# antonilo/unsupervised_detection

Measured on NVIDIA H100. Metric: frame-pairs/sec adversarial train step 256x448, higher is better.
Workload: dtype bf16

## Files before the change

include/cis_b200.h:

```cpp
#ifndef CIS_B200_H_
#define CIS_B200_H_
#include <stdint.h>
#include <stddef.h>

#ifdef __cplusplus
extern "C" {
#endif

typedef void* cis_stream_t;

enum { CIS_OK = 0, CIS_ERR_BAD_ARG = 1, CIS_ERR_UNSUPPORTED = 2, CIS_ERR_CUDA = 3 };
enum { CIS_ACT_NONE = 0, CIS_ACT_ELU = 1, CIS_ACT_LEAKY = 2 };
enum { CIS_MAX_TAPS = 49, CIS_MAX_SRC = 4 };

typedef struct {
  const void* ptr;
  int32_t pitch;
  int32_t c_off;
  int32_t chunks;
  int32_t n_mod;
} CisSrc;

typedef struct {
  int32_t N, H, W;
  int32_t OH, OW;
  int32_t sh, sw;
  int32_t ntaps;
  int16_t dh[CIS_MAX_TAPS];
  int16_t dw[CIS_MAX_TAPS];
  int32_t nsrc;
  CisSrc src[CIS_MAX_SRC];
  const void* wpack;
  int32_t K_pad;
  int32_t BN;
  int32_t n_tiles;
  const float* bias;
  int32_t act;
  float alpha;
  int32_t DH, DW;
  int32_t osh, osw, oa, ob;
  void* out;
  int32_t out_pitch, out_coff, out_ch;
  float* outf;
  int32_t outf_pitch, outf_coff, outf_ch;
  const void* add_pre;
  int32_t add_pre_pitch, add_pre_coff;
  const float* addf_pre;
  int32_t addf_pitch, addf_coff;
  const void* add_post;
  int32_t add_post_pitch, add_post_coff;
  int32_t mode;
  int32_t halo;
  int32_t dil;
  int32_t MT;
  int32_t hoy, hox;
  int32_t ey, ex;
  int32_t splits;
  float* sk_scratch;
  int32_t* sk_counters;
  int32_t nph;
  int32_t ph_tap[5];
  int32_t sk_cluster;
  int32_t nsub;
  struct {
    int32_t tap0, ntaps;
    int32_t hoy, hox;
    int32_t OH, OW, oa, ob;
    const void* wpack;
  } sub[4];
  int32_t nwg;
  int32_t thin;
} CisConv;

typedef struct {
  int32_t N, H, W, OH, OW, sh, sw, ntaps;
  int16_t dh[CIS_MAX_TAPS];
  int16_t dw[CIS_MAX_TAPS];
  int32_t nsrc;
  CisSrc src[CIS_MAX_SRC];
  const void* g;
  int32_t g_pitch, g_coff, g_chunks;
  float* dwp;
  int32_t Cout;
  int32_t K_pad;
  int32_t splits;
  int32_t tma;
  int32_t nh;
  int32_t nwg;
} CisWgrad;

const char* cis_last_error(void);
int cis_version(void);
uint32_t cis_crc32c(uint32_t crc, const void* data, size_t n);
int cis_host_resize_bilinear_legacy(const float* src, int32_t H, int32_t W, int32_t C, float* dst, int32_t OH, int32_t OW);
int cis_host_bgr8_to_rgb_resized(const unsigned char* bgr, int32_t H, int32_t W, float* dst, int32_t OH, int32_t OW);

int cis_conv_igemm(const CisConv* d, cis_stream_t stream);
int cis_conv_s2_phase_plan(const CisConv* d, CisConv* h, int16_t* wk);
int cis_set_persist_mode(int mode);
int cis_conv_wgrad(const CisWgrad* d, cis_stream_t stream);

int cis_pack_weights(const float* w, const int32_t* kmap, int32_t K_pad, int32_t rows, int32_t cout, int32_t sn, const int32_t* nmap,
                     void* wp, cis_stream_t stream);
int cis_pack_weights_tiled(const float* w, const int32_t* kmap, int32_t cin8, int32_t ntaps, int32_t n_tiles, int32_t BN, int32_t cout,
                           int32_t sn, const int32_t* nmap, void* out, int32_t thin, cis_stream_t stream);
int cis_unpack_wgrad(const float* dwp, const int32_t* kmap, int32_t K_pad, int32_t cout, int32_t nsplit, float* dw, const float* colpart,
                     int32_t nblocks, int32_t nch, float* db, int32_t layout, cis_stream_t stream);
int cis_bn_fold(const float* w, const float* bias, const float* gamma, const float* beta, int64_t nw, int32_t cout, float* w_eff,
                float* b_eff, cis_stream_t stream);
int cis_bn_chain(const float* w, const float* bias, const float* gamma, float* dw_eff_to_dw, const float* db_eff, int64_t nw,
                 int32_t cout, float* dbias, float* dgamma, float* dbeta, cis_stream_t stream);

enum { CIS_JOB_PACK = 0, CIS_JOB_PACK_TILED = 1, CIS_JOB_UNPACK = 2, CIS_JOB_BN_FOLD = 3, CIS_JOB_BN_CHAIN = 4 };
typedef struct {
  int32_t kind;
  int32_t i[8];
  int64_t n;
  const void* p[8];
} CisParamJob;
int cis_param_multi(const CisParamJob* jobs_dev, int32_t njobs, int32_t total_blocks, cis_stream_t stream);

int cis_dact_mul(void* g, int32_t g_pitch, int32_t g_coff, const void* y, int32_t y_pitch, int32_t y_coff, const void* res,
                 int32_t res_pitch, int32_t res_coff, int64_t npix, int32_t chunks, int32_t act, float alpha, cis_stream_t stream);
int cis_add_slice(void* dst, int32_t dst_pitch, int32_t dst_coff, const void* src, int32_t src_pitch, int32_t src_coff,
                  int64_t npix_dst, int32_t chunks, int32_t reps, int32_t accumulate, cis_stream_t stream);
int cis_colsum(const void* g, int32_t g_pitch, int32_t g_coff, int64_t npix, int32_t nch, float* part, int32_t nblocks, cis_stream_t stream);

int cis_zero(void* ptr, int64_t nbytes, cis_stream_t stream);

int cis_dact_colsum(void* g, int32_t g_pitch, int32_t g_coff, const void* y, int32_t y_pitch, int32_t y_coff, const void* res,
                    int32_t res_pitch, int32_t res_coff, int64_t npix, int32_t nch, int32_t act, float alpha, float* part, int32_t nblocks,
                    cis_stream_t stream);

int cis_resize_bilinear_bf16(const void* src, int32_t s_pitch, int32_t s_coff, int32_t N, int32_t H, int32_t W, void* dst,
                             int32_t d_pitch, int32_t d_coff, int32_t OH, int32_t OW, int32_t chunks, cis_stream_t stream);
int cis_resize_concat_bf16(const CisSrc* srcs, int32_t nsrc, int32_t N, int32_t H, int32_t W, void* dst, int32_t d_pitch, int32_t d_coff,
                           int32_t OH, int32_t OW, cis_stream_t stream);
int cis_resize_concat_bf16_bwd(const void* ddst, int32_t d_pitch, int32_t d_coff, int32_t N, int32_t OH, int32_t OW, const CisSrc* grads,
                               const int32_t* want, const int32_t* accumulate, int32_t nsrc, int32_t H, int32_t W, cis_stream_t stream);
int cis_resize_bilinear_bf16_bwd(const void* ddst, int32_t d_pitch, int32_t d_coff, int32_t N, int32_t OH, int32_t OW, void* dsrc,
                                 int32_t s_pitch, int32_t s_coff, int32_t H, int32_t W, int32_t chunks, int32_t accumulate,
                                 cis_stream_t stream);
int cis_resize_bilinear_f32(const float* src, int32_t N, int32_t H, int32_t W, int32_t C, float* dst, int32_t OH, int32_t OW,
                            float scale, cis_stream_t stream);
int cis_upsample_nn2x(const void* src, int32_t N, int32_t H, int32_t W, int32_t pitch, void* dst, cis_stream_t stream);
int cis_upsample_nn2x_bwd(const void* ddst, int32_t N, int32_t H, int32_t W, int32_t pitch, void* dsrc, int32_t accumulate,
                          cis_stream_t stream);
int cis_crop_resize_bilinear_f32(const float* src, int32_t Hs, int32_t Ws, int32_t C, int32_t y0, int32_t x0, int32_t ch, int32_t cw, float* dst,
                                 int32_t OH, int32_t OW, cis_stream_t stream);
int cis_crop_resize_flow_f32(const float* src, int32_t Hs, int32_t Ws, int32_t y0, int32_t x0, int32_t ch, int32_t cw, float* dst, int32_t OH,
                             int32_t OW, float s0, float s1, cis_stream_t stream);
int cis_resize_nn_f32(const float* src, int32_t N, int32_t H, int32_t W, int32_t C, float* dst, int32_t OH, int32_t OW,
                      cis_stream_t stream);
enum { CIS_RESIZE_BILINEAR = 0, CIS_RESIZE_NEAREST = 1 };
int cis_resize_f32(const float* src, int32_t N, int32_t H, int32_t W, int32_t C, float* dst, int32_t OH, int32_t OW, int32_t method,
                   int32_t align_corners, cis_stream_t stream);
int cis_resize_f32_bwd(const float* ddst, int32_t N, int32_t OH, int32_t OW, int32_t C, int32_t H, int32_t W, float* dsrc, int32_t method,
                       int32_t align_corners, cis_stream_t stream);

int cis_warp_costvol(const void* c1, int32_t c1_pitch, int32_t c1_coff, const void* c2, int32_t c2_pitch, int32_t c2_coff,
                     const float* flow, float flow_scale, int32_t B, int32_t h, int32_t w, int32_t C, void* out, int32_t out_pitch,
                     int32_t out_coff, cis_stream_t stream);
int cis_warp_costvol_r(const void* c1, int32_t c1_pitch, int32_t c1_coff, const void* c2, int32_t c2_pitch, int32_t c2_coff,
                       const float* flow, float flow_scale, int32_t B, int32_t h, int32_t w, int32_t C, void* out, int32_t out_pitch,
                       int32_t out_coff, int32_t search_range, cis_stream_t stream);
int cis_dense_image_warp(const void* img, int32_t pitch, int32_t coff, const float* flow, float flow_scale, int32_t B, int32_t h,
                         int32_t w, int32_t C, void* out, int32_t out_pitch, cis_stream_t stream);

int cis_pack_f32_to_bf16(const float* src, int64_t npix, int32_t C, float offset, void* dst, int32_t d_pitch, int32_t d_coff,
                         cis_stream_t stream);
int cis_flow_stats(const float* flow, int32_t B, int64_t hw, double* stats, cis_stream_t stream);
int cis_pack_generator_input(const float* image, const float* flow, const double* stats, int32_t B, int64_t hw, void* dst,
                             cis_stream_t stream);
int cis_flow_standardize(const float* flow, const double* stats, int32_t B, int64_t hw, float* out, cis_stream_t stream);
int cis_flow_standardize_bwd(const float* y, const float* dy, const double* stats, int32_t B, int64_t hw, double* scratch, float* dx,
                             cis_stream_t stream);
int cis_masked_epe(const float* pred, const float* gt, const float* mask, int32_t B, int64_t hw, double* scratch, double* out,
                   cis_stream_t stream);

int cis_mask_apply(const float* flow, const float* mask, int32_t B, int64_t hw, void* dst, cis_stream_t stream);
int cis_box_masks(float* mask, int32_t B, int32_t H, int32_t W, int32_t lo_h, int32_t hi_h, int32_t lo_w, int32_t hi_w, int64_t sample_offset,
                  const long long* step, uint64_t seed, cis_stream_t stream);
int cis_charbonnier_sum(const float* gt, const float* pred, const float* mask, int32_t B, int64_t hw, int32_t C, int32_t mask_c, float cbn,
// ... 93 lines not shown
```

unsupervised_detection_b200/_lib.py:

```python
import ctypes as C
import os

_HERE = os.path.dirname(os.path.abspath(__file__))
LIB_PATH = os.path.join(_HERE, os.environ.get('CIS_LIB_NAME', 'libcis_b200.so'))

MAX_TAPS, MAX_SRC = 49, 4
ACT_NONE, ACT_ELU, ACT_LEAKY = 0, 1, 2
RESIZE_BILINEAR, RESIZE_NEAREST = 0, 1


class CisSrc(C.Structure):
    _fields_ = [('ptr', C.c_void_p), ('pitch', C.c_int32), ('c_off', C.c_int32), ('chunks', C.c_int32), ('n_mod', C.c_int32)]


class CisParamJob(C.Structure):
    _fields_ = [('kind', C.c_int32), ('i', C.c_int32 * 8), ('n', C.c_int64), ('p', C.c_void_p * 8)]


JOB_PACK, JOB_PACK_TILED, JOB_UNPACK, JOB_BN_FOLD, JOB_BN_CHAIN = range(5)


class CisSub(C.Structure):
    _fields_ = [('tap0', C.c_int32), ('ntaps', C.c_int32), ('hoy', C.c_int32), ('hox', C.c_int32), ('OH', C.c_int32), ('OW', C.c_int32),
                ('oa', C.c_int32), ('ob', C.c_int32), ('wpack', C.c_void_p)]
# ... 34 lines not shown
    _fields_ = [('flow', C.c_void_p * 5), ('grad', C.c_void_p * 5), ('pitch', C.c_int32 * 5), ('c_off', C.c_int32 * 5),
                ('accumulate', C.c_int32 * 5), ('weight', C.c_float * 5)]


class CisFlowAug(C.Structure):
    _fields_ = [('scale', C.c_float * 2), ('rotate', C.c_float * 2), ('translate', C.c_float * 2), ('rel_scale', C.c_float * 2),
                ('rel_rotate', C.c_float * 2), ('rel_translate', C.c_float * 2), ('color', C.c_float * 2), ('contrast', C.c_float * 2),
                ('brightness', C.c_float), ('gamma', C.c_float * 2), ('noise', C.c_float * 2)]


FLOW_AUG_ROW = 32


_i32, _i64, _f32, _p, _u64 = C.c_int32, C.c_int64, C.c_float, C.c_void_p, C.c_uint64

_PROTOS = {
    'cis_conv_igemm': [C.POINTER(CisConv)],
    'cis_conv_wgrad': [C.POINTER(CisWgrad)],
    'cis_pack_weights': [_p, _p, _i32, _i32, _i32, _i32, _p, _p],
    'cis_pack_weights_tiled': [_p, _p, _i32, _i32, _i32, _i32, _i32, _i32, _p, _p, _i32],
    'cis_unpack_wgrad': [_p, _p, _i32, _i32, _i32, _p, _p, _i32, _i32, _p, _i32],
    'cis_bn_fold': [_p, _p, _p, _p, _i64, _i32, _p, _p],
    'cis_param_multi': [_p, _i32, _i32],
    'cis_bn_chain': [_p, _p, _p, _p, _p, _i64, _i32, _p, _p, _p],
    'cis_dact_mul': [_p, _i32, _i32, _p, _i32, _i32, _p, _i32, _i32, _i64, _i32, _i32, _f32],
    'cis_add_slice': [_p, _i32, _i32, _p, _i32, _i32, _i64, _i32, _i32, _i32],
    'cis_colsum': [_p, _i32, _i32, _i64, _i32, _p, _i32],
    'cis_zero': [_p, _i64],
    'cis_dact_colsum': [_p, _i32, _i32, _p, _i32, _i32, _p, _i32, _i32, _i64, _i32, _i32, _f32, _p, _i32],
    'cis_resize_bilinear_bf16': [_p, _i32, _i32, _i32, _i32, _i32, _p, _i32, _i32, _i32, _i32, _i32],
    'cis_resize_concat_bf16': [C.POINTER(CisSrc), _i32, _i32, _i32, _i32, _p, _i32, _i32, _i32, _i32],
    'cis_resize_concat_bf16_bwd': [_p, _i32, _i32, _i32, _i32, _i32, C.POINTER(CisSrc), C.POINTER(C.c_int32), C.POINTER(C.c_int32), _i32, _i32, _i32],
    'cis_resize_bilinear_bf16_bwd': [_p, _i32, _i32, _i32, _i32, _i32, _p, _i32, _i32, _i32, _i32, _i32, _i32],
    'cis_resize_bilinear_f32': [_p, _i32, _i32, _i32, _i32, _p, _i32, _i32, _f32],
    'cis_upsample_nn2x': [_p, _i32, _i32, _i32, _i32, _p],
    'cis_upsample_nn2x_bwd': [_p, _i32, _i32, _i32, _i32, _p, _i32],
    'cis_crop_resize_bilinear_f32': [_p, _i32, _i32, _i32, _i32, _i32, _i32, _i32, _p, _i32, _i32],
    'cis_crop_resize_flow_f32': [_p, _i32, _i32, _i32, _i32, _i32, _i32, _p, _i32, _i32, _f32, _f32],
    'cis_resize_nn_f32': [_p, _i32, _i32, _i32, _i32, _p, _i32, _i32],
    'cis_resize_f32': [_p, _i32, _i32, _i32, _i32, _p, _i32, _i32, _i32, _i32],
    'cis_resize_f32_bwd': [_p, _i32, _i32, _i32, _i32, _i32, _i32, _p, _i32, _i32],
    'cis_flow_standardize': [_p, _p, _i32, _i64, _p],
    'cis_flow_standardize_bwd': [_p, _p, _p, _i32, _i64, _p, _p],
    'cis_masked_epe': [_p, _p, _p, _i32, _i64, _p, _p],
    'cis_warp_costvol': [_p, _i32, _i32, _p, _i32, _i32, _p, _f32, _i32, _i32, _i32, _i32, _p, _i32, _i32],
    'cis_dense_image_warp': [_p, _i32, _i32, _p, _f32, _i32, _i32, _i32, _i32, _p, _i32],
    'cis_pack_f32_to_bf16': [_p, _i64, _i32, _f32, _p, _i32, _i32],
    'cis_flow_stats': [_p, _i32, _i64, _p],
    'cis_pack_generator_input': [_p, _p, _p, _i32, _i64, _p],
    'cis_mask_apply': [_p, _p, _i32, _i64, _p],
    'cis_box_masks': [_p, _i32, _i32, _i32, _i32, _i32, _i32, _i32, _i64, _p, _u64],
    'cis_charbonnier_sum': [_p, _p, _p, _i32, _i64, _i32, _i32, _f32, _p],
    'cis_cis_loss_fwd': [_p, _p, _p, _i32, _i32, _i32, _i32, _i32, _f32, _p, _p],
    'cis_cis_loss_reduce': [_p, _i32, _i32, _i64, _f32, _p, _p],
    'cis_cis_loss_bwd': [_p, _p, _p, _p, _p, _i32, _i32, _i32, _i32, _i32, _f32, _i32, _p, _p],
    'cis_resize_f32_bwd_to_bf16': [_p, _i32, _i32, _i32, _i32, _i32, _i32, _p, _i32],
    'cis_mask_bwd': [_p, _p, _p, _p, _i32, _i64, _p],
    'cis_abs_sum': [_p, _i64, _p],
    'cis_grad_avg_abs': [_p, _p, _i32, _p],
    'cis_clip_adam': [_p, _p, _p, _p, _i64, _f32, _f32, _f32, _f32, _f32, _f32, _p, _p, _i32, _u64],
    'cis_cast_f32_to_bf16': [_p, _i64, _p],
    'cis_cast_bf16_to_f32': [_p, _i64, _i32, _i32, _i32, _p],
    'cis_cast_bf16_to_f32_scaled': [_p, _i64, _i32, _i32, _i32, _f32, _p],
    'cis_charbonnier_bwd': [_p, _p, _p, _i32, _i64, _i32, _i32, _f32, _p, _p, _p, _p],
    'cis_dense_image_warp_bwd': [_p, _i32, _i32, _p, _f32, _i32, _i32, _i32, _i32, _p, _p, _p, _p],
    'cis_cost_volume_bwd': [_p, _i32, _i32, _p, _i32, _i32, _p, _i32, _i32, _i32, _i32, _p, _p, _p],
    'cis_resize_f32_bwd_to_bf16_scaled': [_p, _i32, _i32, _i32, _i32, _i32, _i32, _p, _i32, _f32],
    'cis_warp_costvol_bwd': [_p, _i32, _i32, _p, _i32, _i32, _p, _f32, _i32, _i32, _i32, _i32, _p, _i32, _i32, _p, _i32, _i32, _p, _i32, _i32,
                             _p, _i32, _i32, _i32, _p, _p, _p],
    'cis_parity_split_bf16': [_p, _i32, _i32, _i32, _i32, _i32, _i32, _p, _i32],
    'cis_flow_multiscale_loss': [C.POINTER(CisFlowPyr), _p, _i32, _i32, _i32, _i32, _i32, _f32, _f32, _i32, _f32, _f32, _p, _p],
    'cis_flow_multiscale_loss_bwd': [C.POINTER(CisFlowPyr), _p, _i32, _i32, _i32, _i32, _i32, _f32, _f32, _i32, _f32, _f32],
    'cis_adam_l2': [_p, _p, _p, _p, _i64, _p, _i32, _f32, _p, _f32, _f32, _f32, _p],
    'cis_unsup_flow_loss': [_p, _p, _p, _i32, _i32, _i32, _p, _p, _p, _p, _p],
    'cis_unsup_flow_loss_bwd': [_p, _p, _p, _i32, _i32, _i32, _p, _p, _f32, _f32, _p],
    'cis_flow_aug_params': [C.POINTER(CisFlowAug), _i32, _i32, _i32, _i64, _p, _u64, _p],
    'cis_flow_augment': [_p, _p, _p, _p, _i32, _i32, _i32, _p, _p, _p],
    'cis_warp_costvol_r': [_p, _i32, _i32, _p, _i32, _i32, _p, _f32, _i32, _i32, _i32, _i32, _p, _i32, _i32, _i32],
    'cis_cost_volume_bwd_r': [_p, _i32, _i32, _p, _i32, _i32, _p, _i32, _i32, _i32, _i32, _p, _p, _p, _i32],
    'cis_warp_costvol_bwd_r': [_p, _i32, _i32, _p, _i32, _i32, _p, _f32, _i32, _i32, _i32, _i32, _p, _i32, _i32, _p, _i32, _i32, _p, _i32, _i32,
                               _p, _i32, _i32, _i32, _p, _p, _p, _i32],
}
EXPORTS = sorted(list(_PROTOS) + ['cis_last_error', 'cis_version', 'cis_set_persist_mode', 'cis_crc32c', 'cis_host_resize_bilinear_legacy',
                                  'cis_host_bgr8_to_rgb_resized', 'cis_conv_s2_phase_plan'])

_lib = None


def load():
    global _lib
    if _lib is None:
        if not os.path.exists(LIB_PATH):
            raise RuntimeError('libcis_b200.so not built: run `python -c "import __graft_entry__ as g; g.build()"` '
                               '(no CPU fallback exists for the product path)')
        lib = C.CDLL(LIB_PATH)
        lib.cis_last_error.restype = C.c_char_p
        lib.cis_version.restype = C.c_int
        lib.cis_set_persist_mode.argtypes = [C.c_int]
        lib.cis_set_persist_mode.restype = C.c_int
        lib.cis_crc32c.argtypes = [C.c_uint32, C.c_void_p, C.c_size_t]
        lib.cis_crc32c.restype = C.c_uint32
        lib.cis_host_resize_bilinear_legacy.argtypes = [C.c_void_p, C.c_int32, C.c_int32, C.c_int32, C.c_void_p, C.c_int32, C.c_int32]
        lib.cis_host_resize_bilinear_legacy.restype = C.c_int
        lib.cis_host_bgr8_to_rgb_resized.argtypes = [C.c_void_p, C.c_int32, C.c_int32, C.c_void_p, C.c_int32, C.c_int32]
        lib.cis_host_bgr8_to_rgb_resized.restype = C.c_int
        lib.cis_conv_s2_phase_plan.argtypes = [C.POINTER(CisConv), C.POINTER(CisConv), C.POINTER(C.c_int16)]
        lib.cis_conv_s2_phase_plan.restype = C.c_int
        for name, args in _PROTOS.items():
            fn = getattr(lib, name)
            fn.argtypes = list(args) + [C.c_void_p]
            fn.restype = C.c_int
        _lib = lib
    return _lib


def check(rc, what=''):
    if rc != 0:
        raise RuntimeError('libcis_b200 %s failed (code %d): %s' % (what, rc, load().cis_last_error().decode()))


def call(name, *args):
    check(getattr(load(), name)(*args), name)
```

unsupervised_detection_b200/csrc/conv_igemm.cu:

```cuda
#include "ptx.cuh"
#include "../../include/cis_b200.h"
#include "common.cuh"
#include <cuda.h>
#include <stdlib.h>
#include <string.h>


namespace cis {

#ifdef CIS_TRACE
__device__ unsigned long long* g_trace = nullptr;
__device__ int g_trace_cap = 0;
#define CIS_TRACE_AT(slot)                                                                                         \
  do {                                                                                                             \
    if (g_trace && blockIdx.x == 0 && blockIdx.y == 0 && blockIdx.z == 0 && (slot) < g_trace_cap) g_trace[(slot)] = clock64(); \
  } while (0)
#else
#define CIS_TRACE_AT(slot) ((void)0)
#endif

static constexpr int kBM = 128;
static constexpr int kBK = 64;
static constexpr int kAStage = kBM * 128;
static constexpr int kThreads = 256;
// ... 1284 lines not shown
      const uint32_t st = tile_base + s * kWStage;
#pragma unroll
      for (int r = rl; r < 64; r += nprod >> 3) {
        const int g = (kb0 + it) * 64 + r;
        const bool rv = g < M;
        int n = 0, h0 = 0, w0 = 0;
        if (rv) {
          const int ow = g % p.OW;
          const int t = g / p.OW;
          h0 = (t % p.OH) * p.sh;
          n = t / p.OH;
          w0 = ow * p.sw;
        }
        const uint32_t dst = st + r * 128 + sw_off;
#pragma unroll
        for (int u = 0; u < 2; ++u) {
          const bool ok = rv && avalid[u];
          const size_t off = ok ? ((size_t)g * p.g_pitch + p.g_coff + (u * 8 + j) * 8) : 0;
          cp_async16(dst + u * kWTile, gp + off, ok ? 16u : 0u);
        }
#pragma unroll
        for (int u = 0; u < 2; ++u) {
          const int h = h0 + bdh[u], w = w0 + bdw[u];
          const bool ok = rv && bvalid[u] && (unsigned)h < (unsigned)p.H && (unsigned)w < (unsigned)p.W;
          const int ne = bnmod[u] ? (n % bnmod[u]) : n;
          const size_t off = ok ? ((size_t)((ne * p.H + h) * p.W + w) * bpitch[u] + bcoff[u]) : 0;
          cp_async16(dst + (2 + u) * kWTile, bptr[u] + off, ok ? 16u : 0u);
        }
      }
      cp_async_commit();
      if (it >= S - 1) {
        cp_async_wait<S - 1>();
        fence_proxy_async();
        mbar_arrive(bar_full + 8 * ((it - (S - 1)) % S));
      }
    }
    cp_async_wait<0>();
    fence_proxy_async();
    for (int it = nkb > S - 1 ? nkb - (S - 1) : 0; it < nkb; ++it) mbar_arrive(bar_full + 8 * (it % S));

    }
    mbar_wait(bar_accum, 0);
    const int co = (warp & 3) * 32 + lane;
    const uint32_t t_row = tile_base + (uint32_t)co * 16;
    const int c_lo = mma_warp == 8 ? (warp >> 2) * 64 : 0, c_hi = mma_warp == 8 ? c_lo + 64 : 128;
    const int kcol0 = blockIdx.x * 128;
#pragma unroll 1
    for (int c0 = c_lo; c0 < c_hi; c0 += 16) {
      float v[16];
      acc_ld16(t_row + (uint32_t)c0 * kAccColBytes, v);
      if (co < p.Cout && kcol0 + c0 < p.K_pad) {
        float4* o = reinterpret_cast<float4*>(p.dwp) + (size_t)blockIdx.y * p.Cout * (p.K_pad / 4) + (size_t)((kcol0 + c0) / 4) * p.Cout + co;
        o[0] = make_float4(v[0], v[1], v[2], v[3]);
        o[p.Cout] = make_float4(v[4], v[5], v[6], v[7]);
        o[2 * p.Cout] = make_float4(v[8], v[9], v[10], v[11]);
        o[3 * p.Cout] = make_float4(v[12], v[13], v[14], v[15]);
      }
    }
  } else {
    const int wtid = tid - mma_warp * 32;
    float acc[128];
    for (int it = 0; it < nkb; ++it) {
      const int s = it % S;
      mbar_wait(bar_full + 8 * s, (uint32_t)((it / S) & 1));
      const uint32_t st = tile_base + s * kWStage;
      const uint32_t alo = desc_lo(st, kWTile), blo = desc_lo(st + 2 * kWTile, kWTile), dhi = desc_hi(1024);
      wg_fence();
#pragma unroll
      for (int k = 0; k < 4; ++k) mma128<128, 1, 1>(acc, alo + 128 * k, dhi, blo + 128 * k, dhi, (uint32_t)kWTile >> 4, (uint32_t)((it | k) != 0));
      wg_commit();
      wg_wait<0>();
      if (wtid == 0) mbar_arrive(bar_empty + 8 * s);
    }
    acc_store<128>(acc, tile_base, wtid);
    mbar_arrive(bar_accum);
  }
}


static constexpr int kWHMaxStages = 6;
struct WgradHaloMaps {
  CUtensorMap g;
  CUtensorMap x[CIS_MAX_SRC];
};
template <int NH> struct WgradHaloCfg {
  static_assert(NH == 16 || NH == 32 || NH == 64, "NH is 16, 32 or 64 output channels");
  static constexpr int kPairs = kMaxAccCols / NH;
  static constexpr uint32_t kGRow = 2 * NH;
  static constexpr uint32_t kGTile = 64 * kGRow;
  static constexpr uint32_t kLayout = NH == 64 ? 1u : NH == 32 ? 2u : 3u;
};

template <int NH, int NWG>
__device__ __forceinline__ void wgrad_halo_wg_pairs(int w, int npairs, int cout, int& qa, int& np, int& hf) {
  constexpr int P = WgradHaloCfg<NH>::kPairs;
  const int nhalf = cout > 64 ? 2 : 1;
  if (NWG == 2 && nhalf == 2) {
    qa = blockIdx.z * P;
    np = min(P, npairs - qa);
    hf = w;
    return;
  }
  const int q0 = (blockIdx.z / nhalf) * (NWG * P);
  const int cnt = min(NWG * P, npairs - q0);
  const int h = NWG == 2 ? (cnt + 1) / 2 : cnt;
  qa = q0 + (w ? h : 0);
  np = w ? cnt - h : h;
  hf = blockIdx.z % nhalf;
}

template <int NH, int NWG>
__global__ void __launch_bounds__(128 * (1 + NWG)) conv_wgrad_halo_kernel(const __grid_constant__ CisWgrad p, const __grid_constant__ WgradHaloMaps maps,
                                                                          const int Wh, const int Hh, const int hoy, const int hox,
                                                                          const int stage_bytes, const int S) {
  using Cfg = WgradHaloCfg<NH>;
  constexpr int P = Cfg::kPairs;
  extern __shared__ uint8_t smem_raw[];
  __shared__ uint64_t bars[2 * kWHMaxStages + 1];
  __shared__ int s_off[CIS_MAX_TAPS + 1];
  const uint32_t tile_base = (smem_u32(smem_raw) + 1023u) & ~1023u;
  const uint32_t bar_full = smem_u32(&bars[0]);
  const uint32_t bar_empty = smem_u32(&bars[kWHMaxStages]);
  const uint32_t bar_accum = smem_u32(&bars[2 * kWHMaxStages]);
  const int tid = threadIdx.x, warp = tid >> 5, lane = tid & 31;
  pdl_launch_dependents();
  if (tid < p.ntaps) s_off[tid] = (p.dh[tid] - hoy) * Wh + (p.dw[tid] - hox);
  if (tid == p.ntaps) s_off[tid] = 0;
  const bool wg_halves = NWG == 2 && p.Cout > 64;
  const int ng = wg_halves ? 2 : 1;
  const int halo_bytes = stage_bytes - ng * (int)Cfg::kGTile;
  const int tiles_x = (p.OW + 7) / 8, tiles_y = (p.OH + 7) / 8;
  const int nkb_total = p.N * tiles_x * tiles_y;
  const int per = (nkb_total + (int)gridDim.y - 1) / (int)gridDim.y;
  const int kb0 = blockIdx.y * per;
  const int nkb = min(per, nkb_total - kb0);
  if (nkb <= 0) return;
  int m_chunks = 0;
  for (int i = 0; i < p.nsrc; ++i) m_chunks += p.src[i].chunks;
  const int nch64 = (m_chunks + 7) / 8;
  const int npairs = (p.ntaps + 1) / 2;
  const int c64 = blockIdx.x;

  if (tid == 128) {
    for (int s = 0; s < S; ++s) {
      mbar_init(bar_full + 8 * s, 1);
      mbar_init(bar_empty + 8 * s, NWG);
    }
    mbar_init(bar_accum, 128 * NWG);
    fence_mbar_init();
  }
  pdl_wait();
  __syncthreads();

  if (warp < 4) {
    if (tid == 0) {
      int c = c64 * 8, si = 0;
      while (si < p.nsrc - 1 && c >= p.src[si].chunks) {
        c -= p.src[si].chunks;
        ++si;
      }
      int nm = p.src[0].n_mod;
      if (si == 1) nm = p.src[1].n_mod;
      if (si == 2) nm = p.src[2].n_mod;
      if (si == 3) nm = p.src[3].n_mod;
      int qa, np, hf0;
      wgrad_halo_wg_pairs<NH, NWG>(0, npairs, p.Cout, qa, np, hf0);
      const int tpi = tiles_x * tiles_y;
      for (int it = 0; it < nkb; ++it) {
        const int s = it % S;
        mbar_wait(bar_empty + 8 * s, (uint32_t)(((it / S) & 1) ^ 1));
        const int kb = kb0 + it;
        const int n = kb / tpi, r = kb - n * tpi;
        const int ty = r / tiles_x, tx = r - ty * tiles_x;
        const uint32_t st = tile_base + s * stage_bytes, bar = bar_full + 8 * s;
        mbar_expect_tx(bar, (uint32_t)(Wh * Hh * 128 + ng * (int)Cfg::kGTile));
        tma_load_4d(st, &maps.x[si], bar, c * 8, tx * 8 + hox, ty * 8 + hoy, nm ? (n % nm) : n);
        for (int h = 0; h < ng; ++h)
          tma_load_4d(st + halo_bytes + h * Cfg::kGTile, &maps.g, bar, (hf0 + h) * 64, tx * 8, ty * 8, n);
      }
    }
    __syncwarp();
    mbar_wait(bar_accum, 0);
    const int r = warp * 32 + lane;
    const int cch = r & 63;
    const uint32_t t_row = tile_base + (uint32_t)r * 16;
    for (int w = 0; w < NWG; ++w) {
      int qa, np, hf;
      wgrad_halo_wg_pairs<NH, NWG>(w, npairs, p.Cout, qa, np, hf);
      for (int q = 0; q < np; ++q) {
        const int t = 2 * (qa + q) + (r >> 6);
        if (t >= p.ntaps) continue;
        const size_t kcol = ((size_t)t * nch64 + c64) * 64 + cch;
#pragma unroll 1
        for (int c0 = 0; c0 < NH && hf * 64 + c0 < p.Cout; c0 += 16) {
          float v[16];
          acc_ld16(t_row + (uint32_t)((w * P + q) * NH + c0) * kAccColBytes, v);
          for (int e = 0; e < 16; ++e) {
            const int co = hf * 64 + c0 + e;
            if (co < p.Cout) p.dwp[((size_t)blockIdx.y * p.Cout + co) * p.K_pad + kcol] = v[e];
          }
        }
      }
    }
  } else {
    const int wg = NWG > 1 ? (warp - 4) >> 2 : 0;
    const int wtid = tid - 128 * (1 + wg);
    int qa, np, hf;
    wgrad_halo_wg_pairs<NH, NWG>(wg, npairs, p.Cout, qa, np, hf);
    np = __shfl_sync(0xffffffffu, np, 0);
    float acc[P][NH];
    const uint32_t ahi = desc_hi((uint32_t)(Wh * 128));
    const uint32_t bhi = (((8 * Cfg::kGRow) >> 4) & 0x3FFF) | (Cfg::kLayout << 30);
    const uint32_t kstep = (uint32_t)(2 * Wh * 128) >> 4;
    const uint32_t g_off = (uint32_t)halo_bytes + (wg_halves ? (uint32_t)wg * Cfg::kGTile : 0u);
    for (int it = 0; it < nkb; ++it) {
      const int s = it % S;
      mbar_wait(bar_full + 8 * s, (uint32_t)((it / S) & 1));
      const uint32_t st = tile_base + s * stage_bytes;
      const uint32_t blo0 = desc_lo(st + g_off, Cfg::kGTile);
      wg_fence();
#pragma unroll
      for (int q = 0; q < P; ++q) {
        if (q < np) {
          const int o0 = s_off[2 * (qa + q)], o1 = s_off[2 * (qa + q) + 1];
          const uint32_t lbo = (uint32_t)((o1 > o0 ? o1 - o0 : 1) * 128);
          const uint32_t alo0 = desc_lo(st + (uint32_t)(o0 * 128), lbo);
#pragma unroll
          for (int k = 0; k < 4; ++k)
            mma128<NH, 1, 1>(acc[q], alo0 + k * kstep, ahi, blo0 + Cfg::kGRow * k, bhi, lbo >> 4, (uint32_t)((it | k) != 0));
        }
      }
      wg_commit();
      wg_wait<0>();
      if (wtid == 0) mbar_arrive(bar_empty + 8 * s);
    }
    if constexpr (NWG > 1) asm volatile("bar.sync 1, %0;" ::"n"(128 * NWG) : "memory");
#pragma unroll
    for (int q = 0; q < P; ++q)
      if (q < np) acc_store<NH>(acc[q], tile_base + (uint32_t)((wg * P + q) * NH) * kAccColBytes, wtid);
    mbar_arrive(bar_accum);
  }
}

}

using namespace cis;

static bool pdl_enabled() {
  static const bool on = !(getenv("CIS_PDL") && atoi(getenv("CIS_PDL")) == 0);
  return on;
}
template <typename... KArgs, typename... Args>
static cudaError_t launch_pdl(void (*kern)(KArgs...), dim3 grid, dim3 block, size_t smem, cudaStream_t st, Args... args) {
  cudaLaunchConfig_t cfg;
  memset(&cfg, 0, sizeof(cfg));
  cfg.gridDim = grid;
  cfg.blockDim = block;
  cfg.dynamicSmemBytes = smem;
  cfg.stream = st;
  cudaLaunchAttribute attr[1];
  attr[0].id = cudaLaunchAttributeProgrammaticStreamSerialization;
  attr[0].val.programmaticStreamSerializationAllowed = 1;
  cfg.attrs = attr;
  cfg.numAttrs = pdl_enabled() ? 1 : 0;
  return cudaLaunchKernelEx(&cfg, kern, KArgs(args)...);
}

template <typename... KArgs, typename... Args>
static cudaError_t launch_pdl_zcluster(void (*kern)(KArgs...), dim3 grid, dim3 block, size_t smem, cudaStream_t st, int cz, Args... args) {
  cudaLaunchConfig_t cfg;
  memset(&cfg, 0, sizeof(cfg));
  cfg.gridDim = grid;
  cfg.blockDim = block;
  cfg.dynamicSmemBytes = smem;
  cfg.stream = st;
  cudaLaunchAttribute attr[2];
  attr[0].id = cudaLaunchAttributeClusterDimension;
  attr[0].val.clusterDim.x = 1;
  attr[0].val.clusterDim.y = 1;
  attr[0].val.clusterDim.z = cz;
  attr[1].id = cudaLaunchAttributeProgrammaticStreamSerialization;
  attr[1].val.programmaticStreamSerializationAllowed = 1;
// ... 298 lines not shown
    const long ncta = (long)g->N * tiles_x * tiles_y * g->n_tiles;
    const int cps = max(1, min(225 * 1024 / smem, 4));
    const double t_mma = MT * 2.0 * BN * nst * 0.25, t_mem = (double)kb * nst / 40.0 + halo / 40.0;
    const double t_cta = fmax(t_mma, t_mem) + (4000.0 + 1500.0 * MT) / cps;
    const double cost = (double)((ncta + (long)nsm * cps - 1) / ((long)nsm * cps)) * cps * t_cta / fmin((double)cps, fmax(1.0, (double)ncta / nsm));
    if (!best_mt || cost < best - 1e-9) {
      best = cost;
      best_mt = MT;
    }
  }
  if (!best_mt || (long)g->N * tiles_x * ((g->OH + 16 * best_mt - 1) / (16 * best_mt)) * g->n_tiles < 296) return false;
  h->halo = 1;
  h->sh = h->sw = 1;
  h->dil = 1;
  h->MT = best_mt;
  h->nwg = 1;
  h->hoy = hoy;
  h->hox = hox;
  h->ey = ey;
  h->ex = ex;
  h->nph = 4;
  for (int q = 0; q < 5; ++q) h->ph_tap[q] = bounds[q];
  h->thin = thin;
  h->splits = 0;
  h->sk_cluster = 0;
  for (int s = 0; s < nst; ++s)
    for (int j = 0; j < 2; ++j) {
      const int i = thin == 8 ? 2 * s + j : s;
      wk[2 * s + j] = (int16_t)(thin == 8 ? (i < nt ? order[i] * 8 : g->K_pad) : order[i] * 16 + 8 * j);
    }
  return true;
}
extern "C" int cis_conv_s2_phase_plan(const CisConv* d, CisConv* h, int16_t* wk) {
  return d && h && wk && !d->halo && s2_phase_plan(d, h, wk) ? 1 : 0;
}

extern "C" int cis_conv_igemm(const CisConv* d, cis_stream_t stream) {
  if (!d || d->ntaps < 1 || d->ntaps > CIS_MAX_TAPS || d->nsrc < 1 || d->nsrc > CIS_MAX_SRC || d->K_pad % 64 != 0 || d->K_pad <= 0 ||
      d->n_tiles < 1 || !d->wpack)
    return cis_set_error(CIS_ERR_BAD_ARG, "cis_conv_igemm: bad descriptor");
  int chunks = 0;
  for (int i = 0; i < d->nsrc; ++i) {
    if ((d->src[i].pitch | d->src[i].c_off) & 7) return cis_set_error(CIS_ERR_BAD_ARG, "cis_conv_igemm: source pitch/c_off must be multiples of 8");
    chunks += d->src[i].chunks;
  }
  if (d->ntaps * chunks * 8 > d->K_pad) return cis_set_error(CIS_ERR_BAD_ARG, "cis_conv_igemm: K_pad smaller than taps*channels");
  if (d->mode == 1 && !d->outf) return cis_set_error(CIS_ERR_BAD_ARG, "cis_conv_igemm: mode 1 needs outf");
  if ((d->add_pre || d->add_post) && (((d->add_pre_pitch | d->add_pre_coff | d->add_post_pitch | d->add_post_coff | d->out_ch) & 7) != 0))
    return cis_set_error(CIS_ERR_BAD_ARG, "cis_conv_igemm: residual slices must be 8-channel aligned");
  cudaStream_t st = (cudaStream_t)stream;
  if (d->halo) {
    if (d->MT < 1 || d->MT > 4 || d->MT * d->BN > kMaxAccCols || d->nwg < 0 || d->nwg > 2 || (d->nwg == 2 && d->BN < 64) || d->dil < 1 ||
        d->sh != 1 || d->sw != 1 || d->ey < 0 || d->ex < 0 ||
        (d->dil > 1 && (d->OH != d->H || d->OW != d->W)) || (d->nph > 1 && (d->nph != 4 || d->dil != 1 || d->ph_tap[0] != 0 || d->ph_tap[4] != d->ntaps)))
      return cis_set_error(CIS_ERR_BAD_ARG, "cis_conv_igemm(halo): bad tile parameters");
    switch (d->BN) {
      case 16: return launch_halo<16, 1>(d, st);
      case 32: return launch_halo<32, 1>(d, st);
      case 64: return d->nwg == 2 ? launch_halo<64, 2>(d, st) : launch_halo<64, 1>(d, st);
      case 128: return d->nwg == 2 ? launch_halo<128, 2>(d, st) : launch_halo<128, 1>(d, st);
      default: return cis_set_error(CIS_ERR_UNSUPPORTED, "cis_conv_igemm: BN must be 16/32/64/128");
    }
  }
  CisConv h;
  int16_t wk[2 * CIS_MAX_TAPS];
  if (s2_phase_plan(d, &h, wk)) {
    switch (h.BN) {
      case 16: return launch_halo<16, 1>(&h, st, wk);
      case 32: return launch_halo<32, 1>(&h, st, wk);
      case 64: return launch_halo<64, 1>(&h, st, wk);
      case 128: return launch_halo<128, 1>(&h, st, wk);
    }
  }
  switch (d->BN) {
    case 16: return launch_fwd<16>(d, st);
    case 32: return launch_fwd<32>(d, st);
    case 64: return launch_fwd<64>(d, st);
    case 128: return launch_fwd<128>(d, st);
    default: return cis_set_error(CIS_ERR_UNSUPPORTED, "cis_conv_igemm: BN must be 16/32/64/128");
  }
}

template <int NH, int NWG>
static int launch_wgrad_halo_t(const CisWgrad* d, cudaStream_t st, int nch64, int Wh, int Hh, int hoy, int hox, int halo_bytes) {
  using Cfg = WgradHaloCfg<NH>;
  const bool wg_halves = NWG == 2 && d->Cout > 64;
  const int stage = halo_bytes + (wg_halves ? 2 : 1) * (int)Cfg::kGTile;
  const int npairs = (d->ntaps + 1) / 2, nhalf = d->Cout > 64 ? 2 : 1;
  const int gz = wg_halves ? (npairs + Cfg::kPairs - 1) / Cfg::kPairs : nhalf * ((npairs + NWG * Cfg::kPairs - 1) / (NWG * Cfg::kPairs));
  int S = (200 * 1024) / stage;
  if (S > kWHMaxStages) S = kWHMaxStages;
  if (S < 2) return cis_set_error(CIS_ERR_UNSUPPORTED, "cis_conv_wgrad(halo): halo does not fit shared memory");
  int smem = S * stage + 1024;
  const int acc_smem = NWG * kMaxAccCols * (int)kAccColBytes + 1024;
  if (smem < acc_smem) smem = acc_smem;
  static int attr_smem = 0;
  if (smem > attr_smem) {
    cudaError_t e = cudaFuncSetAttribute(conv_wgrad_halo_kernel<NH, NWG>, cudaFuncAttributeMaxDynamicSharedMemorySize, smem);
    if (e != cudaSuccess) return cis_set_cuda_error(e, "cudaFuncSetAttribute(conv_wgrad_halo)");
    attr_smem = smem;
  }
  WgradHaloMaps maps;
  memset(&maps, 0, sizeof(maps));
  CisSrc gs;
  gs.ptr = d->g; gs.pitch = d->g_pitch; gs.c_off = d->g_coff; gs.chunks = d->g_chunks; gs.n_mod = 0;
  const CUtensorMapSwizzle gswz = NH == 64 ? CU_TENSOR_MAP_SWIZZLE_128B : NH == 32 ? CU_TENSOR_MAP_SWIZZLE_64B : CU_TENSOR_MAP_SWIZZLE_32B;
  bool ok = encode_src_map(&maps.g, gs, d->N, d->OH, d->OW, 8, 8, 1, 0, 0, 1, NH, gswz);
  for (int i = 0; ok && i < d->nsrc; ++i) ok = encode_src_map(&maps.x[i], d->src[i], d->N, d->H, d->W, Wh, Hh);
  if (!ok) return cis_set_error(CIS_ERR_CUDA, "cis_conv_wgrad(halo): cuTensorMapEncodeTiled failed / unavailable");
  dim3 grid(nch64, d->splits, gz);
  cudaError_t le = launch_pdl(conv_wgrad_halo_kernel<NH, NWG>, grid, dim3(128 * (1 + NWG)), (size_t)smem, st, *d, maps, Wh, Hh, hoy, hox, stage, S);
  if (le != cudaSuccess) return cis_set_cuda_error(le, "launch(conv_wgrad_halo)");
  return cis_check_launch("conv_wgrad_halo");
}

static int launch_wgrad_halo(const CisWgrad* d, cudaStream_t st) {
  if (d->sh != 1 || d->sw != 1) return cis_set_error(CIS_ERR_BAD_ARG, "cis_conv_wgrad(halo): needs a stride-1 layer");
  int chunks = 0;
  for (int i = 0; i < d->nsrc; ++i) chunks += d->src[i].chunks;
  for (int i = 0; i < d->nsrc - 1; ++i)
    if (d->src[i].chunks % 8) return cis_set_error(CIS_ERR_BAD_ARG, "cis_conv_wgrad(halo): needs 64-channel aligned concat sources");
  const int nch64 = (chunks + 7) / 8;
  int hoy = d->dh[0], hox = d->dw[0], my = d->dh[0], mx = d->dw[0];
  for (int t = 1; t < d->ntaps; ++t) {
    if (d->dh[t] < hoy) hoy = d->dh[t];
    if (d->dw[t] < hox) hox = d->dw[t];
    if (d->dh[t] > my) my = d->dh[t];
    if (d->dw[t] > mx) mx = d->dw[t];
  }
  for (int t = 1; t < d->ntaps; ++t)
    if ((d->dh[t] - hoy) * 1024 + (d->dw[t] - hox) <= (d->dh[t - 1] - hoy) * 1024 + (d->dw[t - 1] - hox))
      return cis_set_error(CIS_ERR_BAD_ARG, "cis_conv_wgrad(halo): taps must be listed in increasing row-major order");
  const int Wh = 8 + (mx - hox), Hh = 8 + (my - hoy);
  if (Wh > 256 || Hh > 256) return cis_set_error(CIS_ERR_UNSUPPORTED, "cis_conv_wgrad(halo): tap extent too large");
  if (d->K_pad < d->ntaps * nch64 * 64) return cis_set_error(CIS_ERR_BAD_ARG, "cis_conv_wgrad(halo): K_pad smaller than taps * 64-channel groups");
  const int nh = d->nh ? d->nh : 64, nwg = d->nwg ? d->nwg : 1;
  if ((nh != 16 && nh != 32 && nh != 64) || nh < (d->Cout > 64 ? 64 : (d->Cout + 15) / 16 * 16) || nwg < 1 || nwg > 2)
    return cis_set_error(CIS_ERR_BAD_ARG, "cis_conv_wgrad(halo): nh must be 16/32/64 and cover Cout (64 above 64), nwg 1 or 2");
  const int halo_bytes = (Wh * Hh * 128 + 1023) & ~1023;
  switch (nh * 4 + nwg) {
    case 16 * 4 + 1: return launch_wgrad_halo_t<16, 1>(d, st, nch64, Wh, Hh, hoy, hox, halo_bytes);
    case 16 * 4 + 2: return launch_wgrad_halo_t<16, 2>(d, st, nch64, Wh, Hh, hoy, hox, halo_bytes);
    case 32 * 4 + 1: return launch_wgrad_halo_t<32, 1>(d, st, nch64, Wh, Hh, hoy, hox, halo_bytes);
    case 32 * 4 + 2: return launch_wgrad_halo_t<32, 2>(d, st, nch64, Wh, Hh, hoy, hox, halo_bytes);
    case 64 * 4 + 1: return launch_wgrad_halo_t<64, 1>(d, st, nch64, Wh, Hh, hoy, hox, halo_bytes);
    default: return launch_wgrad_halo_t<64, 2>(d, st, nch64, Wh, Hh, hoy, hox, halo_bytes);
  }
}

extern "C" int cis_conv_wgrad(const CisWgrad* d, cis_stream_t stream) {
  if (!d || d->ntaps < 1 || d->ntaps > CIS_MAX_TAPS || d->nsrc < 1 || d->nsrc > CIS_MAX_SRC || d->K_pad % 64 != 0 || d->Cout < 1 ||
      d->Cout > 128 || d->splits < 1 || !d->g || !d->dwp)
    return cis_set_error(CIS_ERR_BAD_ARG, "cis_conv_wgrad: bad descriptor");
  {
    const long M = (long)d->N * d->OH * d->OW;
    const long nkb_total = d->tma ? (long)d->N * ((d->OW + 7) / 8) * ((d->OH + 7) / 8) : (M + 63) / 64;
    const long per = (nkb_total + d->splits - 1) / d->splits;
    if ((long)(d->splits - 1) * per >= nkb_total) return cis_set_error(CIS_ERR_BAD_ARG, "cis_conv_wgrad: a split would own no reduction block");
  }
  if (d->tma == 2) return launch_wgrad_halo(d, (cudaStream_t)stream);
  static bool attr_set = false;
  if (!attr_set) {
    cudaError_t e = cudaFuncSetAttribute(conv_wgrad_kernel, cudaFuncAttributeMaxDynamicSharedMemorySize, kWSmem);
    if (e != cudaSuccess) return cis_set_cuda_error(e, "cudaFuncSetAttribute(conv_wgrad)");
    attr_set = true;
  }
  WgradMaps maps;
  memset(&maps, 0, sizeof(maps));
  if (d->tma) {
    if (d->sh != 1 || d->sw != 1) return cis_set_error(CIS_ERR_BAD_ARG, "cis_conv_wgrad: TMA path needs a stride-1 layer");
    for (int i = 0; i < d->nsrc - 1; ++i)
      if (d->src[i].chunks % 8) return cis_set_error(CIS_ERR_BAD_ARG, "cis_conv_wgrad: TMA path needs 64-channel aligned concat sources");
    CisSrc gs;
    gs.ptr = d->g; gs.pitch = d->g_pitch; gs.c_off = d->g_coff; gs.chunks = d->g_chunks; gs.n_mod = 0;
    bool ok = encode_src_map(&maps.g, gs, d->N, d->OH, d->OW, 8, 8);
    for (int i = 0; ok && i < d->nsrc; ++i) ok = encode_src_map(&maps.x[i], d->src[i], d->N, d->H, d->W, 8, 8);
    if (!ok) return cis_set_error(CIS_ERR_CUDA, "cis_conv_wgrad: cuTensorMapEncodeTiled failed / unavailable");
  }
  dim3 grid((d->K_pad + 127) / 128, d->splits);
  cudaError_t le = launch_pdl(conv_wgrad_kernel, grid, dim3(d->tma ? kThreads : kGThreads), kWSmem, (cudaStream_t)stream, *d, maps);
  if (le != cudaSuccess) return cis_set_cuda_error(le, "launch(conv_wgrad)");
  return cis_check_launch("conv_wgrad");
}
```

Measured before the change: 661.7.

## Route stride-2 weight-gradient convs through phase-split TMA halo kernel

Adds a stride-2 phase decomposition for weight-gradient convolutions. Taps are regrouped by input parity into four phase planes, each loaded by its own strided TMA tensor map into the halo kernel, which writes results through a per-tap column remap. Stride-2 layers that previously fell to the generic non-TMA wgrad kernel now run on the stride-1 halo path when the plan's constraints are met. This costs four times the halo shared memory per stage, plus padding taps when a phase has an odd tap count.

```diff
diff --git a/include/cis_b200.h b/include/cis_b200.h
--- a/include/cis_b200.h
+++ b/include/cis_b200.h
@@ -99,6 +99,7 @@
 int cis_conv_s2_phase_plan(const CisConv* d, CisConv* h, int16_t* wk);
 int cis_set_persist_mode(int mode);
 int cis_conv_wgrad(const CisWgrad* d, cis_stream_t stream);
+int cis_conv_wgrad_s2_phase_plan(const CisWgrad* d, CisWgrad* h, int16_t* kcol, int32_t* ph_tap);
 
 int cis_pack_weights(const float* w, const int32_t* kmap, int32_t K_pad, int32_t rows, int32_t cout, int32_t sn, const int32_t* nmap,
                      void* wp, cis_stream_t stream);
diff --git a/unsupervised_detection_b200/_lib.py b/unsupervised_detection_b200/_lib.py
--- a/unsupervised_detection_b200/_lib.py
+++ b/unsupervised_detection_b200/_lib.py
@@ -140,7 +140,8 @@
                                _p, _i32, _i32, _i32, _p, _p, _p, _i32],
 }
 EXPORTS = sorted(list(_PROTOS) + ['cis_last_error', 'cis_version', 'cis_set_persist_mode', 'cis_crc32c', 'cis_host_resize_bilinear_legacy',
-                                  'cis_host_bgr8_to_rgb_resized', 'cis_conv_s2_phase_plan'])
+                                  'cis_host_bgr8_to_rgb_resized', 'cis_conv_s2_phase_plan',
+                                  'cis_conv_wgrad_s2_phase_plan'])
 
 _lib = None
 
@@ -164,6 +165,8 @@
         lib.cis_host_bgr8_to_rgb_resized.restype = C.c_int
         lib.cis_conv_s2_phase_plan.argtypes = [C.POINTER(CisConv), C.POINTER(CisConv), C.POINTER(C.c_int16)]
         lib.cis_conv_s2_phase_plan.restype = C.c_int
+        lib.cis_conv_wgrad_s2_phase_plan.argtypes = [C.POINTER(CisWgrad), C.POINTER(CisWgrad), C.POINTER(C.c_int16), C.POINTER(C.c_int32)]
+        lib.cis_conv_wgrad_s2_phase_plan.restype = C.c_int
         for name, args in _PROTOS.items():
             fn = getattr(lib, name)
             fn.argtypes = list(args) + [C.c_void_p]
diff --git a/unsupervised_detection_b200/csrc/conv_igemm.cu b/unsupervised_detection_b200/csrc/conv_igemm.cu
--- a/unsupervised_detection_b200/csrc/conv_igemm.cu
+++ b/unsupervised_detection_b200/csrc/conv_igemm.cu
@@ -1390,6 +1390,9 @@
 struct WgradHaloMaps {
   CUtensorMap g;
   CUtensorMap x[CIS_MAX_SRC];
+  int16_t kcol[CIS_MAX_TAPS];
+  int32_t nph;
+  int32_t ph_tap[5];
 };
 template <int NH> struct WgradHaloCfg {
   static_assert(NH == 16 || NH == 32 || NH == 64, "NH is 16, 32 or 64 output channels");
@@ -1420,7 +1423,7 @@
 template <int NH, int NWG>
 __global__ void __launch_bounds__(128 * (1 + NWG)) conv_wgrad_halo_kernel(const __grid_constant__ CisWgrad p, const __grid_constant__ WgradHaloMaps maps,
                                                                           const int Wh, const int Hh, const int hoy, const int hox,
-                                                                          const int stage_bytes, const int S) {
+                                                                          const int stage_bytes, const int S, const int plane) {
   using Cfg = WgradHaloCfg<NH>;
   constexpr int P = Cfg::kPairs;
   extern __shared__ uint8_t smem_raw[];
@@ -1432,7 +1435,12 @@
   const uint32_t bar_accum = smem_u32(&bars[2 * kWHMaxStages]);
   const int tid = threadIdx.x, warp = tid >> 5, lane = tid & 31;
   pdl_launch_dependents();
-  if (tid < p.ntaps) s_off[tid] = (p.dh[tid] - hoy) * Wh + (p.dw[tid] - hox);
+  const int nph = maps.nph > 1 ? 4 : 1;
+  if (tid < p.ntaps) {
+    int ph = 0;
+    while (ph < nph - 1 && tid >= maps.ph_tap[ph + 1]) ++ph;
+    s_off[tid] = nph > 1 && maps.kcol[tid] < 0 ? 0 : ph * (plane >> 7) + (p.dh[tid] - hoy) * Wh + (p.dw[tid] - hox);
+  }
   if (tid == p.ntaps) s_off[tid] = 0;
   const bool wg_halves = NWG == 2 && p.Cout > 64;
   const int ng = wg_halves ? 2 : 1;
@@ -1481,8 +1489,9 @@
         const int n = kb / tpi, r = kb - n * tpi;
         const int ty = r / tiles_x, tx = r - ty * tiles_x;
         const uint32_t st = tile_base + s * stage_bytes, bar = bar_full + 8 * s;
-        mbar_expect_tx(bar, (uint32_t)(Wh * Hh * 128 + ng * (int)Cfg::kGTile));
-        tma_load_4d(st, &maps.x[si], bar, c * 8, tx * 8 + hox, ty * 8 + hoy, nm ? (n % nm) : n);
+        mbar_expect_tx(bar, (uint32_t)(nph * Wh * Hh * 128 + ng * (int)Cfg::kGTile));
+        for (int ph = 0; ph < nph; ++ph)
+          tma_load_4d(st + ph * plane, &maps.x[si * nph + ph], bar, c * 8, tx * 8 + hox, ty * 8 + hoy, nm ? (n % nm) : n);
         for (int h = 0; h < ng; ++h)
           tma_load_4d(st + halo_bytes + h * Cfg::kGTile, &maps.g, bar, (hf0 + h) * 64, tx * 8, ty * 8, n);
       }
@@ -1498,14 +1507,23 @@
       for (int q = 0; q < np; ++q) {
         const int t = 2 * (qa + q) + (r >> 6);
         if (t >= p.ntaps) continue;
-        const size_t kcol = ((size_t)t * nch64 + c64) * 64 + cch;
+        size_t base = (size_t)blockIdx.y * p.Cout * p.K_pad, cstride = p.K_pad;
+        if (nph > 1) {
+          const int ch = c64 * 64 + cch;
+          if (maps.kcol[t] < 0 || ch >= m_chunks * 8) continue;
+          const int k = maps.kcol[t] + ch;
+          base += (size_t)(k >> 2) * p.Cout * 4 + (k & 3);
+          cstride = 4;
+        } else {
+          base += ((size_t)t * nch64 + c64) * 64 + cch;
+        }
 #pragma unroll 1
         for (int c0 = 0; c0 < NH && hf * 64 + c0 < p.Cout; c0 += 16) {
           float v[16];
           acc_ld16(t_row + (uint32_t)((w * P + q) * NH + c0) * kAccColBytes, v);
           for (int e = 0; e < 16; ++e) {
             const int co = hf * 64 + c0 + e;
-            if (co < p.Cout) p.dwp[((size_t)blockIdx.y * p.Cout + co) * p.K_pad + kcol] = v[e];
+            if (co < p.Cout) p.dwp[base + (size_t)co * cstride] = v[e];
           }
         }
       }
@@ -1970,7 +1988,8 @@
 }
 
 template <int NH, int NWG>
-static int launch_wgrad_halo_t(const CisWgrad* d, cudaStream_t st, int nch64, int Wh, int Hh, int hoy, int hox, int halo_bytes) {
+static int launch_wgrad_halo_t(const CisWgrad* d, cudaStream_t st, int nch64, int Wh, int Hh, int hoy, int hox, int halo_bytes, int plane,
+                               const int16_t* kcol, const int32_t* ph_tap) {
   using Cfg = WgradHaloCfg<NH>;
   const bool wg_halves = NWG == 2 && d->Cout > 64;
   const int stage = halo_bytes + (wg_halves ? 2 : 1) * (int)Cfg::kGTile;
@@ -1994,15 +2013,24 @@
   gs.ptr = d->g; gs.pitch = d->g_pitch; gs.c_off = d->g_coff; gs.chunks = d->g_chunks; gs.n_mod = 0;
   const CUtensorMapSwizzle gswz = NH == 64 ? CU_TENSOR_MAP_SWIZZLE_128B : NH == 32 ? CU_TENSOR_MAP_SWIZZLE_64B : CU_TENSOR_MAP_SWIZZLE_32B;
   bool ok = encode_src_map(&maps.g, gs, d->N, d->OH, d->OW, 8, 8, 1, 0, 0, 1, NH, gswz);
-  for (int i = 0; ok && i < d->nsrc; ++i) ok = encode_src_map(&maps.x[i], d->src[i], d->N, d->H, d->W, Wh, Hh);
+  const int nph = kcol ? 4 : 1;
+  for (int i = 0; ok && i < d->nsrc; ++i)
+    for (int ph = 0; ok && ph < nph; ++ph)
+      ok = encode_src_map(&maps.x[i * nph + ph], d->src[i], d->N, d->H, d->W, Wh, Hh, nph > 1 ? 2 : 1, ph >> 1, ph & 1);
   if (!ok) return cis_set_error(CIS_ERR_CUDA, "cis_conv_wgrad(halo): cuTensorMapEncodeTiled failed / unavailable");
+  maps.nph = nph;
+  if (kcol) {
+    memcpy(maps.kcol, kcol, sizeof(maps.kcol));
+    memcpy(maps.ph_tap, ph_tap, sizeof(maps.ph_tap));
+  }
   dim3 grid(nch64, d->splits, gz);
-  cudaError_t le = launch_pdl(conv_wgrad_halo_kernel<NH, NWG>, grid, dim3(128 * (1 + NWG)), (size_t)smem, st, *d, maps, Wh, Hh, hoy, hox, stage, S);
+  cudaError_t le = launch_pdl(conv_wgrad_halo_kernel<NH, NWG>, grid, dim3(128 * (1 + NWG)), (size_t)smem, st, *d, maps, Wh, Hh, hoy, hox, stage, S,
+                              plane);
   if (le != cudaSuccess) return cis_set_cuda_error(le, "launch(conv_wgrad_halo)");
   return cis_check_launch("conv_wgrad_halo");
 }
 
-static int launch_wgrad_halo(const CisWgrad* d, cudaStream_t st) {
+static int launch_wgrad_halo(const CisWgrad* d, cudaStream_t st, const int16_t* kcol = nullptr, const int32_t* ph_tap = nullptr) {
   if (d->sh != 1 || d->sw != 1) return cis_set_error(CIS_ERR_BAD_ARG, "cis_conv_wgrad(halo): needs a stride-1 layer");
   int chunks = 0;
   for (int i = 0; i < d->nsrc; ++i) chunks += d->src[i].chunks;
@@ -2016,24 +2044,80 @@
     if (d->dh[t] > my) my = d->dh[t];
     if (d->dw[t] > mx) mx = d->dw[t];
   }
-  for (int t = 1; t < d->ntaps; ++t)
+  for (int t = 1; !kcol && t < d->ntaps; ++t)
     if ((d->dh[t] - hoy) * 1024 + (d->dw[t] - hox) <= (d->dh[t - 1] - hoy) * 1024 + (d->dw[t - 1] - hox))
       return cis_set_error(CIS_ERR_BAD_ARG, "cis_conv_wgrad(halo): taps must be listed in increasing row-major order");
   const int Wh = 8 + (mx - hox), Hh = 8 + (my - hoy);
   if (Wh > 256 || Hh > 256) return cis_set_error(CIS_ERR_UNSUPPORTED, "cis_conv_wgrad(halo): tap extent too large");
-  if (d->K_pad < d->ntaps * nch64 * 64) return cis_set_error(CIS_ERR_BAD_ARG, "cis_conv_wgrad(halo): K_pad smaller than taps * 64-channel groups");
+  if (!kcol && d->K_pad < d->ntaps * nch64 * 64) return cis_set_error(CIS_ERR_BAD_ARG, "cis_conv_wgrad(halo): K_pad smaller than taps * 64-channel groups");
   const int nh = d->nh ? d->nh : 64, nwg = d->nwg ? d->nwg : 1;
   if ((nh != 16 && nh != 32 && nh != 64) || nh < (d->Cout > 64 ? 64 : (d->Cout + 15) / 16 * 16) || nwg < 1 || nwg > 2)
     return cis_set_error(CIS_ERR_BAD_ARG, "cis_conv_wgrad(halo): nh must be 16/32/64 and cover Cout (64 above 64), nwg 1 or 2");
-  const int halo_bytes = (Wh * Hh * 128 + 1023) & ~1023;
+  const int plane = (Wh * Hh * 128 + 1023) & ~1023, halo_bytes = (kcol ? 4 : 1) * plane;
   switch (nh * 4 + nwg) {
-    case 16 * 4 + 1: return launch_wgrad_halo_t<16, 1>(d, st, nch64, Wh, Hh, hoy, hox, halo_bytes);
-    case 16 * 4 + 2: return launch_wgrad_halo_t<16, 2>(d, st, nch64, Wh, Hh, hoy, hox, halo_bytes);
-    case 32 * 4 + 1: return launch_wgrad_halo_t<32, 1>(d, st, nch64, Wh, Hh, hoy, hox, halo_bytes);
-    case 32 * 4 + 2: return launch_wgrad_halo_t<32, 2>(d, st, nch64, Wh, Hh, hoy, hox, halo_bytes);
-    case 64 * 4 + 1: return launch_wgrad_halo_t<64, 1>(d, st, nch64, Wh, Hh, hoy, hox, halo_bytes);
-    default: return launch_wgrad_halo_t<64, 2>(d, st, nch64, Wh, Hh, hoy, hox, halo_bytes);
-  }
+    case 16 * 4 + 1: return launch_wgrad_halo_t<16, 1>(d, st, nch64, Wh, Hh, hoy, hox, halo_bytes, plane, kcol, ph_tap);
+    case 16 * 4 + 2: return launch_wgrad_halo_t<16, 2>(d, st, nch64, Wh, Hh, hoy, hox, halo_bytes, plane, kcol, ph_tap);
+    case 32 * 4 + 1: return launch_wgrad_halo_t<32, 1>(d, st, nch64, Wh, Hh, hoy, hox, halo_bytes, plane, kcol, ph_tap);
+    case 32 * 4 + 2: return launch_wgrad_halo_t<32, 2>(d, st, nch64, Wh, Hh, hoy, hox, halo_bytes, plane, kcol, ph_tap);
+    case 64 * 4 + 1: return launch_wgrad_halo_t<64, 1>(d, st, nch64, Wh, Hh, hoy, hox, halo_bytes, plane, kcol, ph_tap);
+    default: return launch_wgrad_halo_t<64, 2>(d, st, nch64, Wh, Hh, hoy, hox, halo_bytes, plane, kcol, ph_tap);
+  }
+}
+
+static bool wgrad_s2_phase_plan(const CisWgrad* g, CisWgrad* h, int16_t* kcol, int32_t* ph_tap) {
+  int chunks = 0;
+  for (int i = 0; i < g->nsrc; ++i) {
+    chunks += g->src[i].chunks;
+    if (i < g->nsrc - 1 && g->src[i].chunks % 8) return false;
+    if (((uintptr_t)g->src[i].ptr + (size_t)g->src[i].c_off * 2) % 16) return false;
+  }
+  const int cin8 = chunks * 8;
+  if (g->tma != 0 || g->sh != 2 || g->sw != 2 || g->nsrc != 1 || (cin8 != 16 && cin8 != 32 && cin8 % 64 != 0) || g->H < 2 || g->W < 2 ||
+      g->K_pad > 32767 || g->ntaps * cin8 > g->K_pad)
+    return false;
+  const int nt = g->ntaps;
+  int order[CIS_MAX_TAPS + 4], bounds[5] = {0, 0, 0, 0, 0}, k = 0;
+  for (int q = 0; q < 4; ++q) {
+    for (int t = 0; t < nt; ++t)
+      if (((g->dh[t] & 1) << 1 | (g->dw[t] & 1)) == q) order[k++] = t;
+    if ((k - bounds[q]) & 1) order[k++] = -1;
+    bounds[q + 1] = k;
+  }
+  if (k > CIS_MAX_TAPS) return false;
+  int hoy = 1 << 20, hox = 1 << 20, my = -(1 << 20), mx = -(1 << 20);
+  for (int t = 0; t < nt; ++t) {
+    hoy = min(hoy, g->dh[t] >> 1);
+    hox = min(hox, g->dw[t] >> 1);
+    my = max(my, g->dh[t] >> 1);
+    mx = max(mx, g->dw[t] >> 1);
+  }
+  const int Wh = 8 + mx - hox, Hh = 8 + my - hoy;
+  const int cout = g->Cout, nh = cout > 64 ? 64 : (cout + 15) / 16 * 16, P = kMaxAccCols / nh, npairs = k / 2;
+  const int nwg = cout > 64 || npairs > P ? 2 : 1;
+  const int plane = (Wh * Hh * 128 + 1023) & ~1023, stage = 4 * plane + (nwg == 2 && cout > 64 ? 2 : 1) * 64 * 2 * nh;
+  if (npairs * nh > 512 || Wh > 256 || Hh > 256 || (200 * 1024) / stage < 2) return false;
+  const long nkb = (long)g->N * ((g->OW + 7) / 8) * ((g->OH + 7) / 8), per = (nkb + g->splits - 1) / g->splits;
+  if ((long)(g->splits - 1) * per >= nkb) return false;
+  const int gz = cout > 64 ? (npairs + P - 1) / P : (npairs + nwg * P - 1) / (nwg * P);
+  if ((long)((cin8 + 63) / 64) * g->splits * gz * 2 < cis_num_sms()) return false;
+  *h = *g;
+  for (int i = 0; i < k; ++i) {
+    const int t = order[i] >= 0 ? order[i] : order[i - 1];
+    h->dh[i] = (int16_t)(g->dh[t] >> 1);
+    h->dw[i] = (int16_t)(g->dw[t] >> 1);
+    kcol[i] = (int16_t)(order[i] >= 0 ? order[i] * cin8 : -1);
+  }
+  for (int i = k; i < CIS_MAX_TAPS; ++i) kcol[i] = -1;
+  h->ntaps = k;
+  h->sh = h->sw = 1;
+  h->tma = 2;
+  h->nh = nh;
+  h->nwg = nwg;
+  for (int q = 0; q < 5; ++q) ph_tap[q] = bounds[q];
+  return true;
+}
+extern "C" int cis_conv_wgrad_s2_phase_plan(const CisWgrad* d, CisWgrad* h, int16_t* kcol, int32_t* ph_tap) {
+  return d && h && kcol && ph_tap && wgrad_s2_phase_plan(d, h, kcol, ph_tap) ? 1 : 0;
 }
 
 extern "C" int cis_conv_wgrad(const CisWgrad* d, cis_stream_t stream) {
@@ -2047,6 +2131,12 @@
     if ((long)(d->splits - 1) * per >= nkb_total) return cis_set_error(CIS_ERR_BAD_ARG, "cis_conv_wgrad: a split would own no reduction block");
   }
   if (d->tma == 2) return launch_wgrad_halo(d, (cudaStream_t)stream);
+  if (!d->tma) {
+    CisWgrad h;
+    int16_t kcol[CIS_MAX_TAPS];
+    int32_t ph_tap[5];
+    if (wgrad_s2_phase_plan(d, &h, kcol, ph_tap)) return launch_wgrad_halo(&h, (cudaStream_t)stream, kcol, ph_tap);
+  }
   static bool attr_set = false;
   if (!attr_set) {
     cudaError_t e = cudaFuncSetAttribute(conv_wgrad_kernel, cudaFuncAttributeMaxDynamicSharedMemorySize, kWSmem);
```

Result: no change. 660.4 (median of 6 runs) (-0.2%).
